# rl-augmented-mpc/Biped-PyMPC

Measured on AMD Instinct MI355X. Metric: batched SRBD QP solves/sec (N=10, 10 PDIPM iters), higher is better.
Workload: dtype f64; 1 GPU; SRBD MPC QP step: qp_former + 10-iteration sparse PDIPM, batch 4096/GPU, horizon N=10, standing gait; batch_per_gpu=4096, global_batch=4096, horizon=10, pdipm_iters=10, refinement=adaptive, parallelism=dp1

## Files before the change

### biped_pympc_amd/_native.py

```python
from __future__ import annotations

import ctypes
import os

from biped_pympc_amd.build import LIB_DIR

_LIB_NAME = "libsrbd_mpc.so"
_lib = None

_c_dp = ctypes.c_void_p


class NativeLibraryMissing(RuntimeError):
    pass


def lib_path() -> str:
    return os.environ.get("SRBD_LIB") or os.path.join(LIB_DIR, _LIB_NAME)


def lib() -> ctypes.CDLL:
    global _lib
    if _lib is not None:
        return _lib
# ... 44 lines not shown
    L.srbd_scratch_pool_slots.restype = ctypes.c_int
    L.srbd_scratch_pool_slots.argtypes = []
    L.srbd_scratch_slot_bytes.restype = ctypes.c_size_t
    L.srbd_scratch_slot_bytes.argtypes = []
    L.srbd_evaluate_qp_former.restype = ctypes.c_float
    L.srbd_evaluate_qp_former.argtypes = [ctypes.c_int, ctypes.c_void_p, ctypes.c_void_p,
                                          ctypes.c_void_p, ctypes.c_int]
    L.srbd_evaluate_pdipm.restype = ctypes.c_float
    L.srbd_evaluate_pdipm.argtypes = [ctypes.c_int, ctypes.c_int, ctypes.c_void_p, ctypes.c_void_p,
                                      ctypes.c_void_p, ctypes.c_int]
    L.srbd_set_solver_path.restype = ctypes.c_int
    L.srbd_set_solver_path.argtypes = [ctypes.c_int]
    L.srbd_get_solver_path.restype = ctypes.c_int
    L.srbd_get_solver_path.argtypes = []
    L.srbd_set_refinement.restype = ctypes.c_int
    L.srbd_set_refinement.argtypes = [ctypes.c_int]
    L.srbd_get_refinement.restype = ctypes.c_int
    L.srbd_get_refinement.argtypes = []
    L.srbd_set_refinement_policy.restype = ctypes.c_int
    L.srbd_set_refinement_policy.argtypes = [ctypes.c_int, ctypes.c_double]
    L.srbd_pattern_ccs.restype = ctypes.c_int
    L.srbd_pattern_ccs.argtypes = [ctypes.c_int, ctypes.c_int, ctypes.POINTER(ctypes.c_int),
                                   ctypes.POINTER(ctypes.c_int)]
    L.srbd_prepare_inputs.restype = ctypes.c_int
    L.srbd_prepare_inputs.argtypes = [ctypes.c_int, ctypes.c_int, ctypes.POINTER(MPCPrep), P, ctypes.c_void_p]
    L.srbd_mpc_step.restype = ctypes.c_int
    L.srbd_mpc_step.argtypes = [ctypes.c_int, ctypes.c_int, ctypes.c_int, ctypes.c_double, ctypes.POINTER(MPCPrep),
                                P, P, _c_dp, ctypes.c_int, _c_dp, _c_dp, _c_dp, ctypes.c_void_p]
    L.srbd_mpc_step_ex.restype = ctypes.c_int
    L.srbd_mpc_step_ex.argtypes = L.srbd_mpc_step.argtypes[:-1] + [_c_dp, ctypes.c_void_p]
    L.srbd_u0_wrench.restype = ctypes.c_int
    L.srbd_u0_wrench.argtypes = [ctypes.c_int, ctypes.c_int, _c_dp, _c_dp, _c_dp, ctypes.c_void_p]
    L.srbd_u0_wrench_torque.restype = ctypes.c_int
    L.srbd_u0_wrench_torque.argtypes = [ctypes.c_int, ctypes.c_int, _c_dp, _c_dp, _c_dp, ctypes.c_int, _c_dp,
                                        _c_dp, _c_dp, ctypes.c_void_p]
    L.srbd_dense_scatter.restype = ctypes.c_int
    L.srbd_dense_scatter.argtypes = [ctypes.c_int, ctypes.c_int, ctypes.c_int, _c_dp, _c_dp, _c_dp,
                                     ctypes.c_void_p]
    _lib = L
    return L


class _Tolerant:

    class _Missing:
        def __init__(self, name):
# ... 153 lines not shown
```

### biped_pympc_amd/csrc/pdipm_srbd_reg.hpp

```cpp
#pragma once
#include "pdipm_srbd.hpp"
#include "qp_former.hpp"
#include "mpc_io.hpp"

#ifndef SRBD_PROGRESS_PRIO
#define SRBD_PROGRESS_PRIO 1
#endif
#ifndef SRBD_PHASE_ATTR
#define SRBD_PHASE_ATTR
#endif
#ifndef SRBD_REFINE_COMBINED
#define SRBD_REFINE_COMBINED 0
#endif
#ifndef SRBD_SWP_INV
#define SRBD_SWP_INV 0
#endif

namespace srbd {

__host__ __device__ constexpr int reg_tpb(int N) { return N <= 10 ? 64 : (N <= 21 ? 128 : (N <= 24 ? 192 : 256)); }
__host__ __device__ constexpr bool reg_horizon(int N) { return N >= 2 && N <= 32; }

template <int TPB>
__device__ __forceinline__ void qp_sync() {
// ... 214 lines not shown
}
template <bool kForce = true>
__device__ __forceinline__ double ncol(const double* nd, int col, const double* v, int p) {
  double a0 = nd[nd_idx(0, col)] * v[0] + nd[nd_idx(1, col)] * v[1];
  double a1 = nd[nd_idx(2, col)] * v[2] + nd[nd_idx(6, col)] * v[6];
  double a2 = nd[nd_idx(7, col)] * v[7] + nd[nd_idx(8, col)] * v[8];
  if (kForce) {
    a0 += nd[nd_idx(3 + p, col)] * v[3 + p];
    a1 += nd[nd_idx(9 + p, col)] * v[9 + p];
  }
  return (a0 + a1) + a2;
}

__host__ __device__ constexpr int g_other(int k) { return k < 2 ? 0 : (k < 4 ? 1 : (k < 6 ? 3 : 0)); }

__host__ __device__ constexpr int g_row(int k) { return 4 * k + kGfPad * (k >> 3); }

__device__ __forceinline__ double grow4(const double* gf, int k, const double* xu) {
  const int f = k >> 3, o = g_other(k & 7);
  const double* g = gf + g_row(k);
  return g[o] * xu[foot_colj(f, o)] + g[2] * xu[foot_colj(f, 2)];
}

template <int N, bool kFReg = true>
struct RegCtx {
  static constexpr int TPB = reg_tpb(N);
  using Lo = RegLayout<N>;
  static constexpr int nz = Lo::nz, m = Lo::m, p = Lo::p, nx = Lo::nx;
  static constexpr int SI = Lo::SI, SE = Lo::SE, SX = Lo::SX;
  static_assert(6 * N <= TPB && 2 * N <= TPB, "equality-row slots");
  struct ERow {
    int e, i, r;
    bool valid;
  };
  __device__ static ERow erow(int l, int t) {
    ERow q;
    if (t == 2) {
      q.valid = l < 2 * N;
      q.e = nx + l;
      q.i = l >> 1;
      q.r = l & 1;
      return q;
    }
    q.valid = l < 6 * N;
    q.i = div6(l);
    const int k = l - m24(q.i, 6);
// ... 66 lines not shown
  }
  __device__ bool block_any_or_all(bool p, bool q) {
    if constexpr (TPB == 64) return __any(p) || !__any(!q);
    else return block_reduce<true>(p ? -1.0 : (q ? 1.0 : 0.0)) != 0.0;
  }
  __device__ double block_min(double v) { return block_reduce<true>(v); }
  __device__ int fresh_lane() const {
    int l = lane;
    asm volatile("" : "+v"(l));
    __builtin_assume(l < TPB);
    return l;
  }
  __device__ static constexpr bool full_slot(int t, int n) { return TPB * (t + 1) <= n; }

  template <int t>
  __device__ double arow(const double* V, const double* Mc, const double* Pd, const double* Nd, const ERow& q) const {
    const double mv = mrow_slot<t>(Mc, q.r, V + 12 * (q.i >= 1 ? q.i - 1 : 0));
    double v = (q.i >= 1 ? 1.0 : 0.0) * mv;
    v += Pd[q.r] * V[12 * q.i + q.r];
    v += nrow<t>(Nd, q.r, V + nx + 12 * q.i);
    return v;
  }
  __device__ static int sink(bool valid, int e, int base) { return valid ? e : Lo::DMY - base; }
  template <int t>
  __device__ void re_slot(const double* X, const double* Mc, const double* Pd, const double* Nd,
                          const double (&bv)[SE]) {
    const ERow q = erow(fresh_lane(), t);
    re[t] = arow<t>(X, Mc, Pd, Nd, q) - bv[t];
  }
  template <int t>
  __device__ void g_slot(const double* TV, const double* Mc, const double* Pd, const double* Nd, double* QV) {
    const ERow q = erow(fresh_lane(), t);
    QV[sink(q.valid, q.e, Lo::QV)] = arow<t>(TV, Mc, Pd, Nd, q) + re[t];
  }
  SRBD_PHASE_ATTR __device__ double residuals(bool want_mu) {
    const int lane = fresh_lane();
    const double *X = at(Lo::X), *Y = at(Lo::Y), *Z = at(Lo::Z), *Mc = at(Lo::Mc), *Nd = at(Lo::Nd),
                 *Gf = at(Lo::Gf), *Pd = at(Lo::Pd), *Hu = at(Lo::Hu), *SG = at(Lo::SG);
    double *RXu = at(Lo::RXu), *REm = at(Lo::REm);
    const double(&fx)[SX] = fxr, (&fu)[SX] = fur, (&bv)[SE] = bvr, (&hv)[SI] = hvr;
#pragma unroll
    for (int t = 0; t < SX; ++t) {
      const int c = lane + TPB * t;
      if (full_slot(t, nx) || c < nx) {
        const int k = div12(c) + 1, j = c - m24(k - 1, 12);
        const double v = Hu[12 + j] * X[c] + ((kFReg || t == 0) ? fx[t] : fg()[c]);
        double ay = Pd[j] * Y[12 * (k - 1) + j];
        const double my = mcol(Mc, j, Y + 12 * (k < N ? k : N - 1));
        ay = fma(k < N ? 1.0 : 0.0, my, ay);
        rxx[t] = v + ay;
      }
    }
#pragma unroll
    for (int t = 0; t < SX; ++t) {
      const int c = lane + TPB * t;
      if (full_slot(t, nx) || c < nx) {
        const int i = div12(c), j = c - m24(i, 12);
        const double v = Hu[j] * X[nx + c] + ((kFReg || t == 0) ? fu[t] : fg()[nx + c]);
        const int fj = foot_of(j), f = fj >= 0 ? fj : 0;
        const double* zf = Z + 16 * i + 8 * f;
        const double* g = Gf + g_row(8 * f) + foot_pos(j);
        double g0 = 0.0, g1 = 0.0;
#pragma unroll
        for (int k = 0; k < 4; ++k) {
          g0 += g[4 * k] * zf[k];
          g1 += g[4 * (k + 4)] * zf[k + 4];
        }
        const double gz = (fj >= 0 ? 1.0 : 0.0) * (g0 + g1);
        double ay = ncol(Nd, j, Y + 12 * i, j % 3);
        const bool e9 = j == 9;
        const double se = (j == 6 || e9) ? 1.0 : 0.0;
        ay = fma(se * (e9 ? SG[7] : SG[6]), Y[nx + 2 * i + (e9 ? 1 : 0)], ay);
        RXu[c] = (v + gz) + ay;
      }
    }
    re_slot<0>(X, Mc, Pd, Nd, bv);
    re_slot<1>(X, Mc, Pd, Nd, bv);
    {
      const ERow q = erow(lane, 2);
      if (q.valid) {
        const int w = q.r;
        re[2] = SG[6 + w] * X[nx + 12 * q.i + (w ? 9 : 6)] - (kFReg ? bv[2] : bg()[q.e]);
        REm[q.e - nx] = re[2];
      }
    }
    double sz = 0.0;
#pragma unroll
    for (int t = 0; t < SI; ++t) {
      const int q = lane + TPB * t;
      if (RegCtx<N>::full_slot(t, m) || q < m) {
        const int i = q >> 4, k = q & 15;
        const double v = grow4(Gf, k, X + nx + m24(i, 12));
        rs[t] = (v + s[t]) - ((kFReg || t < SI - 1) ? hv[t] : hg()[q]);
        sz += s[t] * z[t];
      }
    }
    qp_sync<TPB>();
    return want_mu ? block_sum(sz) / m : 0.0;
  }

  __device__ static double fwd_rhs(bool act, bool prev, bool mstep, int g, int r, const CoupleRow& Cr, double w,
                                   const double* qv) {
    double q = 0.0;
    if (act && !(mstep && g == 1)) q = *qv;
    if (act && prev) q = couple_cw_sub(Cr, w, q);
    if (mstep && nb >= 1) q += __shfl(q, 16 + perm12(r), 64);
    return q;
  }

  __device__ void factor() {
    factor_build();
    factor_chain<false>();
  }

  __device__ void foot_inverse(int fl, double* dst) {
// ... 195 lines not shown
        }
        if constexpr (kFwd) {
          const double q = fwd_rhs(act, prev, mstep, g, r, Cr, wf, QV + 12 * i + pr);
          if (act && !(mstep && g == 1)) {
            wf = dot_bc12(Dr, q);
            QV[12 * i + pr] = wf;
          }
        }
      }
    }
    qp_sync<TPB>();
    PROF_ADD(2);
  }

  template <int kMode>
  __device__ void solve(double smu, bool rx = false, bool step0 = true) {
    solve_rhs<kMode>(smu, rx);
    solve_chain<false>();
    solve_finish<false, false, true>(step0);
  }

  template <int t, bool kPark>
  __device__ void rho_slot(const double* TV, const double* Mc, const double* Pd, const double* Nd, double* QV,
                           double* DYs) {
    const ERow q = erow(fresh_lane(), t);
    const double v = arow<t>(TV, Mc, Pd, Nd, q);
    const int e = sink(q.valid, q.e, Lo::QV);
    const double dy = QV[e];
    if (kPark) DYs[sink(q.valid, q.e, Lo::RXu)] = dy;
    QV[e] = (v + re[t]) - kDelta * dy;
  }
  template <bool kAff = false>
  SRBD_PHASE_ATTR __device__ void refine_rhs(bool row1 = true) {
    const int lane = fresh_lane();
    const double *Mc = at(Lo::Mc), *Nd = at(Lo::Nd), *Pd = at(Lo::Pd), *Gf = at(Lo::Gf), *Hu = at(Lo::Hu);
    double *TV = at(Lo::TV), *QV = at(Lo::QV), *DYs = at(Lo::RXu), *Zd = at(Lo::Z);
    if constexpr (kAff) {
      double *VV = at(Lo::VV);
#pragma unroll
      for (int t = 0; t < SI; ++t) {
        const int q = lane + TPB * t;
        e3r[t] = 0.0;
        if (RegCtx<N>::full_slot(t, m) || q < m) {
          const int i = q >> 4, k = q & 15;
          const double gd = grow4(Gf, k, TV + nx + m24(i, 12));
          const double e3 = -rs[t] - ((gd + ds[t]) - kDelta * dz[t]);
          const double e2 = Zd[q] - (wd[t] * ds[t] + dz[t]);
          const double qc = di[t] * (e2 - wd[t] * e3);
          VV[q] = VV[q] + qc;
          e3r[t] = e3;
          Zd[q] = dz[t] + qc;
        }
      }
    }
    qp_sync<TPB>();
    const int fl = lane;
    if (row1 && (unsigned)fl < 2u * N) {
      const int i = fl >> 1, f = fl & 1, b = 12 * i;
      const double* zf = Zd + 16 * i + 8 * f;
      const double* RXu = DYs;
      const double* g = Gf + g_row(8 * f);
      double gt[4];
      {
        double zk[8];
#pragma unroll
        for (int k = 0; k < 8; ++k) zk[k] = zf[k];
        gt[0] = g[0] * zk[0] + g[4] * zk[1];
        gt[1] = g[9] * zk[2] + g[13] * zk[3];
// ... 3 lines not shown
        for (int k = 0; k < 4; ++k) {
          gz0 += g[4 * k + 2] * zk[k];
          gz1 += g[4 * (k + 4) + 2] * zk[k + 4];
        }
        gt[2] = gz0 + gz1;
      }
      double e1[4], c[4];
#pragma unroll
      for (int a = 0; a < 4; ++a) {
        const int j = foot_colj(f, a);
        const double ay = a < 3 ? ncol(Nd, j, QV + b, a) : ncol<false>(Nd, j, QV + b, 0);
        e1[a] = ((-RXu[b + j] - (Hu[j] + kBeta) * TV[nx + b + j]) - gt[a]) - ay;
      }
      phi_solve(fl, e1, c);
#pragma unroll
      for (int a = 0; a < 4; ++a) TV[nx + b + foot_colj(f, a)] += c[a];
    }
    qp_sync<TPB>();
    if (kAff) {
#pragma unroll
      for (int t = 0; t < SI; ++t)
        if (full_slot(t, m) || lane + TPB * t < m) Zd[lane + TPB * t] = e3r[t];
    }
    rho_slot<0, !kAff>(TV, Mc, Pd, Nd, QV, DYs);
    rho_slot<1, !kAff>(TV, Mc, Pd, Nd, QV, DYs);
    qp_sync<TPB>();
    PROF_ADD(6);
  }

  template <int kMode>
  SRBD_PHASE_ATTR __device__ void solve_rhs(double smu, bool rx = false) {
    const int lane = fresh_lane();
    double *VV = at(Lo::VV), *TV = at(Lo::TV), *QV = at(Lo::QV), *Zr2 = at(Lo::Z);
    const double *RXu = at(Lo::RXu), *REm = at(Lo::REm), *IX = at(Lo::IX), *Gf = at(Lo::Gf),
                 *SG = at(Lo::SG), *Mc = at(Lo::Mc), *Nd = at(Lo::Nd), *Pd = at(Lo::Pd);
#pragma unroll
    for (int t = 0; t < SI; ++t) {
      const int q = lane + TPB * t;
      if (RegCtx<N>::full_slot(t, m) || q < m) {
        const double si = rcp3(s[t]);
        double r2 = -(si * (s[t] * z[t]));
        if (kMode == 1) r2 = r2 + -(si * (s[t] * z[t] + ds[t] * dz[t] - smu));
        Zr2[q] = r2;
        VV[q] = di[t] * (r2 + wd[t] * rs[t]);
      }
    }
#pragma unroll
    for (int t = 0; t < SX; ++t) {
      const int c = lane + TPB * t;
      if ((kMode == 0 || rx) && (full_slot(t, nx) || c < nx)) TV[c] = -rxx[t] * IX[c - m24(div12(c), 12)];
    }
    qp_sync<TPB>();
    rhs_tasks<kMode>(lane, rx);
    qp_sync<TPB>();
    g_slot<0>(TV, Mc, Pd, Nd, QV);
    g_slot<1>(TV, Mc, Pd, Nd, QV);
    qp_sync<TPB>();
    PROF_ADD(3);
  }

  template <int kMode>
  __device__ void rhs_tasks(int fl, bool rx) {
    double* TV = at(Lo::TV);
    const double *VV = at(Lo::VV), *RXu = at(Lo::RXu), *REm = at(Lo::REm), *Gf = at(Lo::Gf), *SG = at(Lo::SG);
    if ((unsigned)fl < (unsigned)(((kMode == 0 || rx) ? 3 : 2) * N)) {
      if (fl < 2 * N) {
        const int i = fl >> 1, f = fl & 1, b = 12 * i;
        double rv[4], tv[4];
        {
          const double* vv = VV + 16 * i + 8 * f;
          const double* g = Gf + g_row(8 * f);
          double vk[8];
#pragma unroll
          for (int k = 0; k < 8; ++k) vk[k] = vv[k];
          const double gfx = g[0] * vk[0] + g[4] * vk[1];
          const double gfy = g[9] * vk[2] + g[13] * vk[3];
          const double gmy = g[19] * vk[4] + g[23] * vk[5];
          double gz0 = 0.0, gz1 = 0.0;
#pragma unroll
// ... 85 lines not shown
      }
#pragma unroll
      for (int te = T - 1; te >= 0; --te) {
        if (te < cnt) {
          const int i = g ? N - 1 - te : te;
          double Dr[12];
#pragma unroll
          for (int k = 0; k < 12; ++k) Dr[k] = dv_at(DV, offs[k], 2 * kDvBytes * te);
          y = dot_bc12_sub(Dr, couple_cty2(Ct, y), wv[te]);
          if (own) QV[12 * i + pr] = y;
        }
      }
    }
    qp_sync<TPB>();
    PROF_ADD(4);
  }

  template <bool kRefine = false, bool kAffine = false, bool kStep0 = false>
  SRBD_PHASE_ATTR __device__ void solve_finish(bool step0 = true) {
    const int lane = fresh_lane();
    double *VV = at(Lo::VV), *TV = at(Lo::TV), *QV = at(Lo::QV), *DYm = at(Lo::DYm);
    const double *RXu = at(Lo::RXu), *REm = at(Lo::REm), *IX = at(Lo::IX), *Gf = at(Lo::Gf),
                 *SG = at(Lo::SG), *Mc = at(Lo::Mc), *Nd = at(Lo::Nd), *Pd = at(Lo::Pd);
#pragma unroll
    for (int t = 0; t < SX; ++t) {
      const int c = lane + TPB * t;
      if (!kAffine && (full_slot(t, nx) || c < nx)) {
        const int k = div12(c) + 1, j = c - m24(k - 1, 12);
        double aty = Pd[j] * QV[12 * (k - 1) + j];
        const double mq = mcol(Mc, j, QV + 12 * (k < N ? k : N - 1));
        aty = fma(k < N ? 1.0 : 0.0, mq, aty);
        TV[c] = TV[c] - aty * IX[j];
      }
    }
    const int fl = lane;
    if ((unsigned)fl < (unsigned)((kAffine ? 2 : 3) * N)) {
      const bool foot = kAffine || fl < 2 * N;
      const int i = foot ? (fl >> 1) : fl - 2 * N;
      const int b = nx + 12 * i;
      const double* yi = QV + 12 * i;
      if (foot) {
        const int f = fl & 1;
        double av[4], tv[4];
#pragma unroll
        for (int a = 0; a < 3; ++a) av[a] = ncol(Nd, foot_colj(f, a), yi, a);
        av[3] = ncol<false>(Nd, foot_colj(f, 3), yi, 0);
        phi_solve(fl, av, tv);
#pragma unroll
        for (int a = 0; a < 4; ++a) {
          const int o = b + foot_colj(f, a);
          TV[o] = TV[o] - tv[a];
        }
      } else {
        const double r4a = kRefine ? 0.0 : -REm[2 * i], r4b = kRefine ? 0.0 : -REm[2 * i + 1];
        const double a6 = ncol<false>(Nd, 6, yi, 0), a9 = ncol<false>(Nd, 9, yi, 0);
        const double a8 = ncol<false>(Nd, 8, yi, 0), a11 = ncol<false>(Nd, 11, yi, 0);
        TV[b + 6] -= SG[0] * a6;
        TV[b + 9] -= SG[2] * a9;
        TV[b + 8] -= SG[1] * a8;
        TV[b + 11] -= SG[3] * a11;
        if constexpr (kRefine) {
          DYm[2 * i] -= (SG[6] * a6) * SG[8];
          DYm[2 * i + 1] -= (SG[7] * a9) * SG[9];
        } else {
          const double rho6 = -RXu[12 * i + 6] - a6, rho9 = -RXu[12 * i + 9] - a9;
          DYm[2 * i] = (SG[6] * rho6 - SG[4] * r4a) * SG[8];
          DYm[2 * i + 1] = (SG[7] * rho9 - SG[5] * r4b) * SG[9];
        }
      }
    }
    qp_sync<TPB>();
#pragma unroll
    for (int t = 0; t < SI; ++t) {
      const int q = lane + TPB * t;
      if (RegCtx<N>::full_slot(t, m) || q < m) {
        const int i = q >> 4, k = q & 15;
        const double gd = grow4(Gf, k, TV + nx + m24(i, 12));
        const double vq = VV[q];
        dz[t] = vq + di[t] * wd[t] * gd;
        const double r3 = (kRefine && kAffine) ? at(Lo::Z)[q] - rs[t] : -rs[t];
        ds[t] = r3 - gd + kDelta * dz[t];
        if (kStep0 && step0) {
          double* Zd = at(Lo::Z);
          const double e3 = -rs[t] - ((gd + ds[t]) - kDelta * dz[t]);
          const double e2 = Zd[q] - (wd[t] * ds[t] + dz[t]);
          const double qc = di[t] * (e2 - wd[t] * e3);
          VV[q] = vq + qc;
          rs[t] = rs[t] - e3;
          Zd[q] = dz[t] + qc;
        }
      }
    }
    PROF_ADD(3);
  }

  __device__ double step_length(const double (&v)[SI], const double (&dv)[SI]) {
    const int lane = fresh_lane();
    double mn = INFINITY;
#pragma unroll
    for (int t = 0; t < SI; ++t) {
// ... 526 lines not shown
```

### biped_pympc_amd/csrc/srbd_mpc.hip

```cpp
#include <hip/hip_runtime.h>

#include <algorithm>
#include <cstdio>
#include <cstdlib>
#include <cstring>
#include <mutex>
#include <shared_mutex>
#include <string>
#include <vector>

#include "../../include/srbd_mpc.h"
#include "pdipm.hpp"
#include "pdipm_srbd.hpp"
#include "pdipm_srbd_reg.hpp"
#include "mpc_step_lds.hpp"
#include "qp_former.hpp"
#include "mpc_io.hpp"
#include "reg20.hpp"
#include "regN.hpp"
#include "device_state.hpp"

#ifndef SRBD_BUILD_ID
#define SRBD_BUILD_ID "0000000000000000"
#endif
// ... 226 lines not shown
  Events* ev = events.at(current_device());
  if (!ev) {
    set_error((int)hipErrorInvalidDevice, "no current HIP device (or index >= 64)");
    return -1.0f;
  }
  if (!ev->ev[0]) {
    if (hipEventCreate(&ev->ev[0]) != hipSuccess || hipEventCreate(&ev->ev[1]) != hipSuccess) {
      set_error((int)hipErrorInitializationError, "hipEventCreate");
      return -1.0f;
    }
  }
  (void)hipEventRecord(ev->ev[0], 0);
  if (launch() != 0) return -1.0f;
  (void)hipEventRecord(ev->ev[1], 0);
  hipError_t e = hipEventSynchronize(ev->ev[1]);
  if (e == hipSuccess) e = hipDeviceSynchronize();
  if (e != hipSuccess) {
    set_error((int)e, "kernel execution");
    return -1.0f;
  }
  float ms = 0.0f;
  (void)hipEventElapsedTime(&ms, ev->ev[0], ev->ev[1]);
  return ms / 1000.0f;
}

}

extern "C" {

int srbd_abi_version(void) { return SRBD_ABI_VERSION; }

const char* srbd_build_id(void) { return kBuildIdTag + sizeof("srbd-build-id:") - 1; }

const char* srbd_last_error(void) { return g_last_error.c_str(); }

size_t srbd_solver_lds_bytes(int horizon) { return horizon_ok(horizon) ? solver_lds_bytes(horizon) : 0; }

int srbd_set_solver_path(int path) {
  if (path < 0 || path > 2)
    return set_error(kErrInvalid, "srbd_set_solver_path: 0 (auto), 1 (general) or 2 (LDS-resident fast)");
  int* p = g_solver_path.at(current_device());
  if (!p) return set_error((int)hipErrorInvalidDevice, "srbd_set_solver_path: no current HIP device");
  *p = path;
  return 0;
}

// ... 311 lines not shown
      a.prep.out[i] = former_inputs[i];
    }
  a.ctrl = 1;
  if (outputs)
    for (int i = 0; i < 6; ++i) a.out[i] = outputs[i];
  a.wrench = foot_wrench;
  a.tau = tau;
  a.jac = contact_jacobian;
  a.contact = contact_bool;
  a.ndof = tau ? ndof : 0;
  a.N = horizon;
  a.n_iter = n_iter;
  a.batch = batch;
  a.y0 = y0;
  a.status = status;
  return launch_step(a, (hipStream_t)stream);
}

int srbd_mpc_step(int horizon, int n_iter, int batch, double y0, const srbd_mpc_prep* prep,
                  double* const* former_inputs, double* const* outputs, float* foot_wrench, int ndof,
                  const float* contact_jacobian, const float* contact_bool, float* tau, void* stream) {
  return srbd_mpc_step_ex(horizon, n_iter, batch, y0, prep, former_inputs, outputs, foot_wrench, ndof,
                          contact_jacobian, contact_bool, tau, nullptr, stream);
}

int srbd_pattern_ccs(int horizon, int which, int* colptr, int* rowind) {
  if (!horizon_ok(horizon) || !colptr || !rowind) return -1;
  constexpr srbd::Tables T = srbd::make_tables();
  const int N = horizon, nz = 24 * N;
  int nnz = 0;
  std::vector<int> row, col;
  auto put = [&](int off, int r, int c) {
    if (off < 0 || off >= nnz) return false;
    if (row[off] != -1) return false;
    row[off] = r;
    col[off] = c;
    return true;
  };
  if (which == 0) {
    nnz = nz;
    row.assign(nnz, -1);
    col.assign(nnz, -1);
    for (int c = 0; c < nz; ++c)
      if (!put(c, c, c)) return -2;
  } else if (which == 1) {
    nnz = srbd::nnz_A(N);
// ... 89 lines not shown
```

### include/srbd_mpc.h

```cpp
#ifndef SRBD_MPC_H_
#define SRBD_MPC_H_

#include <stddef.h>

#ifdef __cplusplus
extern "C" {
#endif

#define SRBD_ABI_VERSION 1
#define SRBD_MAX_HORIZON 32

float evaluate(const double* inputs[], double* work, double* outputs[], const int batch_size);

int srbd_abi_version(void);
const char* srbd_last_error(void);
const char* srbd_build_id(void);

float srbd_evaluate_qp_former(int horizon, const double* inputs[], double* work, double* outputs[],
                              int batch);
float srbd_evaluate_pdipm(int horizon, int n_iter, const double* inputs[], double* work,
                          double* outputs[], int batch);

int srbd_qp_former(int horizon, int batch, const double* const* inputs, double* const* outputs,
                   void* stream);
// ... 29 lines not shown
int srbd_get_solver_path(void);

int srbd_set_refinement(int mode);
int srbd_get_refinement(void);

#define SRBD_REFINE_AFFINE_ALL 1
#define SRBD_REFINE_AFFINE_AT_INIT 2
#define SRBD_REFINE_AFFINE_FIRST(k) (((k) & 255) << 8)
#define SRBD_REFINE_AFFINE_LAST(k) (((k) & 255) << 16)
int srbd_set_refinement_policy(int flags, double w);

int srbd_prepare_device(void);

int srbd_release_device(void);

int srbd_set_scratch_slots(int slots);

size_t srbd_scratch_pool_bytes(void);
int srbd_scratch_pool_slots(void);
size_t srbd_scratch_slot_bytes(void);

int srbd_pattern_ccs(int horizon, int which, int* colptr, int* rowind);


typedef struct srbd_mpc_prep {
  const float* root_euler;
  const float* root_position;
  const float* root_angular_velocity_w;
  const float* root_velocity_w;
  const float* rotation_body;
  const float* foot_position;
  const float* desired_velocity_b;
  const float* desired_angular_velocity_b;
  const float* desired_height;
  float* world_position_desired;
  float* yaw_desired;
  unsigned char* first_run;
  const float* gait_phase;
  const int* ssp_durations;
  const int* dsp_durations;
  const float* contact_table;
  const float* dt_mpc;
  const float* residual_lin_accel;
  const float* residual_ang_accel;
  float I_body[9];
  double mass, mu;
// ... 34 lines not shown
```

Before: 6.747 million solves/s.

## Replace per-lane index arithmetic with constant-memory byte-offset lane tables

```diff
diff --git a/biped_pympc_amd/_native.py b/biped_pympc_amd/_native.py
--- a/biped_pympc_amd/_native.py
+++ b/biped_pympc_amd/_native.py
@@ -90,6 +90,8 @@
     L.srbd_pattern_ccs.restype = ctypes.c_int
     L.srbd_pattern_ccs.argtypes = [ctypes.c_int, ctypes.c_int, ctypes.POINTER(ctypes.c_int),
                                    ctypes.POINTER(ctypes.c_int)]
+    L.srbd_lane_table.restype = ctypes.c_int
+    L.srbd_lane_table.argtypes = [ctypes.c_int, ctypes.c_int, ctypes.POINTER(ctypes.c_uint), ctypes.c_int]
     L.srbd_prepare_inputs.restype = ctypes.c_int
     L.srbd_prepare_inputs.argtypes = [ctypes.c_int, ctypes.c_int, ctypes.POINTER(MPCPrep), P, ctypes.c_void_p]
     L.srbd_mpc_step.restype = ctypes.c_int
diff --git a/biped_pympc_amd/csrc/pdipm_srbd_reg.hpp b/biped_pympc_amd/csrc/pdipm_srbd_reg.hpp
--- a/biped_pympc_amd/csrc/pdipm_srbd_reg.hpp
+++ b/biped_pympc_amd/csrc/pdipm_srbd_reg.hpp
@@ -260,6 +260,267 @@
   return g[o] * xu[foot_colj(f, o)] + g[2] * xu[foot_colj(f, 2)];
 }
 
+#ifndef SRBD_LANE_TABLES
+#define SRBD_LANE_TABLES 1
+#endif
+
+__device__ __forceinline__ double lds_off(const double* base, uint32_t off) {
+  return *reinterpret_cast<const double*>(reinterpret_cast<const char*>(base) + off);
+}
+__device__ __forceinline__ double& lds_off(double* base, uint32_t off) {
+  return *reinterpret_cast<double*>(reinterpret_cast<char*>(base) + off);
+}
+
+constexpr int kGRowTabRows = 16 * 32;
+struct GRowTab {
+  alignas(16) uint32_t o[kGRowTabRows][4];
+};
+__host__ __device__ constexpr uint32_t grow_ref(int q, int w) {
+  const int i = q >> 4, k = q & 15, f = k >> 3, o = g_other(k & 7);
+  return (uint32_t)(8 * (w == 0 ? g_row(k) + o : (w == 1 ? g_row(k) + 2 : 12 * i + foot_colj(f, w == 2 ? o : 2))));
+}
+constexpr GRowTab make_grow_tab() {
+  GRowTab t{};
+  int q = 0;
+  for (int i = 0; i < 32; ++i)
+    for (int f = 0; f < 2; ++f)
+      for (int k = 0; k < 8; ++k, ++q) {
+        const int row = 4 * (8 * f + k) + kGfPad * f;
+        const int oth = k < 2 ? 0 : (k < 4 ? 1 : (k < 6 ? 3 : 0));
+        const int co = oth < 3 ? oth + 3 * f : 7 + 3 * f, cz = 2 + 3 * f;
+        t.o[q][0] = (uint32_t)(8 * (row + oth));
+        t.o[q][1] = (uint32_t)(8 * (row + 2));
+        t.o[q][2] = (uint32_t)(8 * (12 * i + co));
+        t.o[q][3] = (uint32_t)(8 * (12 * i + cz));
+      }
+  return t;
+}
+constexpr bool grow_tab_ok() {
+  const GRowTab t = make_grow_tab();
+  for (int q = 0; q < kGRowTabRows; ++q)
+    for (int w = 0; w < 4; ++w)
+      if (t.o[q][w] != grow_ref(q, w)) return false;
+  return true;
+}
+static_assert(grow_tab_ok(), "c_growtab differs from grow4's index arithmetic");
+static __constant__ GRowTab c_growtab = make_grow_tab();
+
+template <class T>
+__device__ __forceinline__ T ctab_load(const void* base, uint32_t off) {
+  return *reinterpret_cast<const T*>(reinterpret_cast<const char*>(base) + off);
+}
+__device__ __forceinline__ double grow4_tab(const double* gf, const uint4& o, const double* u) {
+  return lds_off(gf, o.x) * lds_off(u, o.z) + lds_off(gf, o.y) * lds_off(u, o.w);
+}
+
+constexpr uint32_t kOneHi = 0x3FF0u;
+
+constexpr int kUColTabRows = 12 * 32 + 128;
+struct UColTab {
+  alignas(16) uint32_t a[kUColTabRows][4];
+  alignas(16) uint32_t b[kUColTabRows][4];
+  alignas(16) uint32_t c[kUColTabRows][4];
+};
+__host__ __device__ constexpr uint32_t ucol_ref(int c, int w) {
+  const int i = c / 12, j = c % 12;
+  const int fj = (j < 3 || j == 7) ? 0 : ((j < 6 || j == 10) ? 1 : -1), f = fj >= 0 ? fj : 0;
+  const int pos = j < 6 ? j % 3 : 3, p = j % 3, e9 = j == 9 ? 1 : 0;
+  switch (w) {
+    case 0: return (uint32_t)(8 * j);
+    case 1: return (uint32_t)(8 * 12 * i);
+    case 2: return (uint32_t)(8 * (16 * i + 8 * f));
+    case 3: return (uint32_t)(8 * (g_row(8 * f) + pos));
+    case 4: return (uint32_t)(8 * nd_idx(3 + p, j));
+    case 5: return (uint32_t)(8 * (12 * i + 3 + p));
+    case 6: return ((fj >= 0 ? kOneHi : 0u) << 16) | ((j == 6 || j == 9) ? kOneHi : 0u);
+    case 7: return 0u;
+    case 8: return (uint32_t)(8 * (6 + e9));
+    default: return (uint32_t)(8 * (2 * i + e9));
+  }
+}
+constexpr UColTab make_ucol_tab() {
+  UColTab tb{};
+  constexpr int foot[12] = {0, 0, 0, 1, 1, 1, -1, 0, -1, -1, 1, -1}, posn[12] = {0, 1, 2, 0, 1, 2, 3, 3, 3, 3, 3, 3},
+                m3[12] = {0, 1, 2, 0, 1, 2, 0, 1, 2, 0, 1, 2};
+  int i = 0, j = 0;
+  for (int c = 0; c < kUColTabRows; ++c) {
+    const int f = foot[j] > 0 ? 1 : 0;
+    tb.a[c][0] = (uint32_t)(8 * j);
+    tb.a[c][1] = (uint32_t)(96 * i);
+    tb.a[c][2] = (uint32_t)(128 * i + 64 * f);
+    tb.a[c][3] = (uint32_t)(8 * ((32 + kGfPad) * f + posn[j]));
+    tb.b[c][0] = (uint32_t)(8 * (kNdS * (3 + m3[j]) + j));
+    tb.b[c][1] = (uint32_t)(96 * i + 24 + 8 * m3[j]);
+    tb.b[c][2] = (foot[j] >= 0 ? kOneHi << 16 : 0u) | ((j == 6 || j == 9) ? kOneHi : 0u);
+    tb.b[c][3] = 0u;
+    tb.c[c][0] = (uint32_t)(j == 9 ? 56 : 48);
+    tb.c[c][1] = (uint32_t)(16 * i + (j == 9 ? 8 : 0));
+    if (++j == 12) {
+      j = 0;
+      ++i;
+    }
+  }
+  return tb;
+}
+constexpr bool ucol_tab_ok() {
+  const UColTab tb = make_ucol_tab();
+  for (int c = 0; c < kUColTabRows; ++c)
+    for (int w = 0; w < 10; ++w)
+      if ((w < 4 ? tb.a[c][w] : (w < 8 ? tb.b[c][w - 4] : tb.c[c][w - 8])) != ucol_ref(c, w)) return false;
+  return true;
+}
+static_assert(ucol_tab_ok(), "c_ucoltab differs from the u-column pass's index arithmetic");
+static __constant__ UColTab c_ucoltab = make_ucol_tab();
+struct UColOffs {
+  uint4 a, b;
+  uint2 c;
+};
+
+template <int N>
+struct ERowTab {
+  static constexpr int TPB = reg_tpb(N);
+  alignas(16) uint32_t a[2][TPB][4];
+  alignas(16) uint32_t b[2][TPB][4];
+  alignas(16) uint32_t c[2][TPB][4];
+};
+template <int N>
+__host__ __device__ constexpr uint32_t erow_ref(int l, int t, int w) {
+  using Lo = RegLayout<N>;
+  const int i = l / 6, k = l % 6, ip = i >= 1 ? i - 1 : 0;
+  const int r = t == 0 ? (k < 3 ? k : k + 3) : (k < 3 ? k + 3 : k + 6);
+  const int rr = t == 0 ? (r < 3 ? r : 0) : (r < 6 ? r : 3);
+  const bool valid = l < 6 * N, ws = t == 0 ? r < 3 : r < 6;
+  const int e = 12 * i + r;
+  switch (w) {
+    case 0: return (uint32_t)(8 * e);
+    case 1: return (uint32_t)(8 * (12 * ip + r));
+    case 2: return (uint32_t)(8 * (12 * ip + (t == 0 ? 0 : rr + 6)));
+    case 3: return (uint32_t)(8 * (12 * i + (t == 0 ? 0 : r % 3)));
+    case 4: return (uint32_t)(8 * r);
+    case 5: return (uint32_t)(8 * (t == 0 ? 12 + 3 * rr : 21 + rr - 3));
+    case 6: return (uint32_t)(8 * nd_idx(r, t == 0 ? 0 : r % 3));
+    case 7: return ((i >= 1 ? kOneHi : 0u) << 16) | (ws ? kOneHi : 0u);
+    case 8: return (uint32_t)(8 * (valid ? e : Lo::DMY - Lo::QV));
+    default: return (uint32_t)(8 * (valid ? e : Lo::DMY - Lo::RXu));
+  }
+}
+template <int N>
+constexpr ERowTab<N> make_erow_tab() {
+  using Lo = RegLayout<N>;
+  ERowTab<N> tb{};
+  for (int t = 0; t < 2; ++t) {
+    int i = 0, k = 0;
+    for (int l = 0; l < ERowTab<N>::TPB; ++l) {
+      const int r = (k < 3 ? k : k + 3) + 3 * t;
+      const int p3 = k < 3 ? k : k - 3;
+      const bool ws = k < 3;
+      const int rr = ws ? r : 3 * t;
+      const int vi = 96 * i, vp = i >= 1 ? vi - 96 : 0;
+      tb.a[t][l][0] = (uint32_t)(vi + 8 * r);
+      tb.a[t][l][1] = (uint32_t)(vp + 8 * r);
+      tb.a[t][l][2] = (uint32_t)(vp + (t == 0 ? 0 : 8 * (rr + 6)));
+      tb.a[t][l][3] = (uint32_t)(vi + (t == 0 ? 0 : 8 * p3));
+      tb.b[t][l][0] = (uint32_t)(8 * r);
+      tb.b[t][l][1] = (uint32_t)(t == 0 ? 96 + 24 * rr : 8 * (18 + rr));
+      tb.b[t][l][2] = (uint32_t)(8 * kNdS * r + (t == 0 ? 0 : 8 * p3));
+      tb.b[t][l][3] = ((i >= 1 ? kOneHi : 0u) << 16) | (ws ? kOneHi : 0u);
+      const bool valid = i < N;
+      tb.c[t][l][0] = valid ? tb.a[t][l][0] : (uint32_t)(8 * (Lo::DMY - Lo::QV));
+      tb.c[t][l][1] = valid ? tb.a[t][l][0] : (uint32_t)(8 * (Lo::DMY - Lo::RXu));
+      if (++k == 6) {
+        k = 0;
+        ++i;
+      }
+    }
+  }
+  return tb;
+}
+template <int N>
+constexpr bool erow_tab_ok() {
+  const ERowTab<N> tb = make_erow_tab<N>();
+  for (int t = 0; t < 2; ++t)
+    for (int l = 0; l < ERowTab<N>::TPB; ++l)
+      for (int w = 0; w < 10; ++w) {
+        const uint32_t v = w < 4 ? tb.a[t][l][w] : (w < 8 ? tb.b[t][l][w - 4] : tb.c[t][l][w - 8]);
+        if (v != erow_ref<N>(l, t, w)) return false;
+      }
+  return true;
+}
+template <int N>
+struct ERowTabHolder {
+  static_assert(erow_tab_ok<N>(), "c_erowtab differs from erow / arow / sink's index arithmetic");
+  static constexpr ERowTab<N> value = make_erow_tab<N>();
+};
+template <int N>
+static __constant__ ERowTab<N> c_erowtab = ERowTabHolder<N>::value;
+
+struct ERowOffs {
+  uint4 a, b;
+  uint2 c;
+};
+
+template <int N>
+struct XColTab {
+  static constexpr int TPB = reg_tpb(N), rows = TPB * RegLayout<N>::SX;
+  alignas(16) uint32_t a[rows][4];
+  alignas(16) uint32_t b[rows][4];
+};
+template <int N>
+__host__ __device__ constexpr uint32_t xcol_ref(int c, int w) {
+  const int k = c / 12 + 1, j = c - 12 * (k - 1), kc = k < N ? k : N - 1;
+  const bool b6 = j >= 6 && j < 9, b9 = j >= 9;
+  const int j6 = b6 ? j - 6 : 0, j9 = b9 ? j - 9 : 0;
+  switch (w) {
+    case 0: return (uint32_t)(8 * j);
+    case 1: return (uint32_t)(8 * (12 * kc + j));
+    case 2: return (uint32_t)(8 * 12 * kc);
+    case 3: return (uint32_t)(8 * (12 * kc + j9 + 3));
+    case 4: return (uint32_t)(8 * j6);
+    case 5: return (uint32_t)(8 * j9);
+    case 6: return ((b6 ? kOneHi : 0u) << 16) | (b9 ? kOneHi : 0u);
+    default: return (k < N ? kOneHi : 0u) << 16;
+  }
+}
+template <int N>
+constexpr XColTab<N> make_xcol_tab() {
+  XColTab<N> tb{};
+  int s = 0, j = 0;
+  for (int c = 0; c < XColTab<N>::rows; ++c) {
+    const int vk = 96 * (s + 1 < N ? s + 1 : N - 1);
+    tb.a[c][0] = (uint32_t)(8 * j);
+    tb.a[c][1] = (uint32_t)(vk + 8 * j);
+    tb.a[c][2] = (uint32_t)vk;
+    tb.a[c][3] = (uint32_t)(vk + (j >= 9 ? 8 * (j - 6) : 24));
+    tb.b[c][0] = (uint32_t)(j >= 6 && j < 9 ? 8 * (j - 6) : 0);
+    tb.b[c][1] = (uint32_t)(j >= 9 ? 8 * (j - 9) : 0);
+    tb.b[c][2] = j >= 9 ? kOneHi : (j >= 6 ? kOneHi << 16 : 0u);
+    tb.b[c][3] = s + 1 < N ? kOneHi << 16 : 0u;
+    if (++j == 12) {
+      j = 0;
+      ++s;
+    }
+  }
+  return tb;
+}
+template <int N>
+constexpr bool xcol_tab_ok() {
+  const XColTab<N> tb = make_xcol_tab<N>();
+  for (int c = 0; c < XColTab<N>::rows; ++c)
+    for (int w = 0; w < 8; ++w)
+      if ((w < 4 ? tb.a[c][w] : tb.b[c][w - 4]) != xcol_ref<N>(c, w)) return false;
+  return true;
+}
+template <int N>
+struct XColTabHolder {
+  static_assert(xcol_tab_ok<N>(), "c_xcoltab differs from the x-column passes' index arithmetic");
+  static constexpr XColTab<N> value = make_xcol_tab<N>();
+};
+template <int N>
+static __constant__ XColTab<N> c_xcoltab = XColTabHolder<N>::value;
+struct XColOffs {
+  uint4 a, b;
+};
+
 template <int N, bool kFReg = true>
 struct RegCtx {
   static constexpr int TPB = reg_tpb(N);
@@ -372,16 +633,90 @@
     return v;
   }
   __device__ static int sink(bool valid, int e, int base) { return valid ? e : Lo::DMY - base; }
+  static constexpr bool kTab = SRBD_LANE_TABLES != 0 && TPB == 64;
+  template <bool kSink>
+  __device__ static ERowOffs load_erow(int l, int t) {
+    const uint32_t off = (uint32_t)l * 16u;
+    ERowOffs o;
+    o.a = ctab_load<uint4>(c_erowtab<N>.a[t], off);
+    o.b = ctab_load<uint4>(c_erowtab<N>.b[t], off);
+    if constexpr (kSink) o.c = ctab_load<uint2>(c_erowtab<N>.c[t], off);
+    else o.c = make_uint2(0u, 0u);
+    return o;
+  }
+  __device__ static uint4 load_grow(int l, int t) {
+    static_assert(TPB * SI <= kGRowTabRows, "c_growtab covers every slot of every lane");
+    return ctab_load<uint4>(c_growtab.o[TPB * t], (uint32_t)l * 16u);
+  }
+  __device__ static XColOffs load_xcol(int l, int t) {
+    const uint32_t off = (uint32_t)l * 16u;
+    return {ctab_load<uint4>(c_xcoltab<N>.a[TPB * t], off), ctab_load<uint4>(c_xcoltab<N>.b[TPB * t], off)};
+  }
+  __device__ static UColOffs load_ucol(int l, int t) {
+    static_assert(TPB * SX <= kUColTabRows, "c_ucoltab covers every slot of every lane");
+    const uint32_t off = (uint32_t)l * 16u;
+    return {ctab_load<uint4>(c_ucoltab.a[TPB * t], off), ctab_load<uint4>(c_ucoltab.b[TPB * t], off),
+            ctab_load<uint2>(c_ucoltab.c[TPB * t], off)};
+  }
+  template <bool kHi>
+  __device__ static double tab_weight(uint32_t w) {
+    return __hiloint2double((int)(kHi ? w & 0xFFFF0000u : w << 16), 0);
+  }
+  __device__ static double mcol_tab(const double* Mc, const double* V, const XColOffs& o) {
+    const double a = lds_off(Mc, o.a.x) * lds_off(V, o.a.y);
+    const double x6 = (lds_off(Mc + 12, o.b.x) * lds_off(V, o.a.z) + lds_off(Mc + 15, o.b.x) * lds_off(V + 1, o.a.z)) +
+                      lds_off(Mc + 18, o.b.x) * lds_off(V + 2, o.a.z);
+    const double x9 = lds_off(Mc + 21, o.b.y) * lds_off(V, o.a.w);
+    return fma(tab_weight<false>(o.b.z), x9, fma(tab_weight<true>(o.b.z), x6, a));
+  }
+  template <int t>
+  __device__ static double arow_tab(const double* V, const double* Mc, const double* Pd, const double* Nd,
+                                    const ERowOffs& o) {
+    const double wi = tab_weight<true>(o.b.w), ws = tab_weight<false>(o.b.w);
+    const double a = lds_off(Mc, o.b.x) * lds_off(V, o.a.y);
+    double x;
+    if constexpr (t == 0)
+      x = (lds_off(Mc, o.b.y) * lds_off(V + 6, o.a.z) + lds_off(Mc + 1, o.b.y) * lds_off(V + 7, o.a.z)) +
+          lds_off(Mc + 2, o.b.y) * lds_off(V + 8, o.a.z);
+    else
+      x = lds_off(Mc, o.b.y) * lds_off(V, o.a.z);
+    const double mv = fma(ws, x, a);
+    double v = wi * mv;
+    v += lds_off(Pd, o.b.x) * lds_off(V, o.a.x);
+    const double* U = V + nx;
+    if constexpr (t == 0) {
+      double a0 = 0.0, a1 = 0.0, a2 = 0.0;
+#pragma unroll
+      for (int j = 0; j < 4; ++j) {
+        a0 += lds_off(Nd + j, o.b.z) * lds_off(U + j, o.a.w);
+        a1 += lds_off(Nd + j + 4, o.b.z) * lds_off(U + j + 4, o.a.w);
+        a2 += lds_off(Nd + j + 8, o.b.z) * lds_off(U + j + 8, o.a.w);
+      }
+      v += (a0 + a1) + a2;
+    } else {
+      v += lds_off(Nd, o.b.z) * lds_off(U, o.a.w) + lds_off(Nd + 3, o.b.z) * lds_off(U + 3, o.a.w);
+    }
+    return v;
+  }
   template <int t>
   __device__ void re_slot(const double* X, const double* Mc, const double* Pd, const double* Nd,
-                          const double (&bv)[SE]) {
-    const ERow q = erow(fresh_lane(), t);
-    re[t] = arow<t>(X, Mc, Pd, Nd, q) - bv[t];
+                          const double (&bv)[SE], const ERowOffs& o) {
+    if constexpr (kTab) {
+      re[t] = arow_tab<t>(X, Mc, Pd, Nd, o) - bv[t];
+    } else {
+      const ERow q = erow(fresh_lane(), t);
+      re[t] = arow<t>(X, Mc, Pd, Nd, q) - bv[t];
+    }
   }
   template <int t>
-  __device__ void g_slot(const double* TV, const double* Mc, const double* Pd, const double* Nd, double* QV) {
-    const ERow q = erow(fresh_lane(), t);
-    QV[sink(q.valid, q.e, Lo::QV)] = arow<t>(TV, Mc, Pd, Nd, q) + re[t];
+  __device__ void g_slot(const double* TV, const double* Mc, const double* Pd, const double* Nd, double* QV,
+                         const ERowOffs& o) {
+    if constexpr (kTab) {
+      lds_off(QV, o.c.x) = arow_tab<t>(TV, Mc, Pd, Nd, o) + re[t];
+    } else {
+      const ERow q = erow(fresh_lane(), t);
+      QV[sink(q.valid, q.e, Lo::QV)] = arow<t>(TV, Mc, Pd, Nd, q) + re[t];
+    }
   }
   SRBD_PHASE_ATTR __device__ double residuals(bool want_mu) {
     const int lane = fresh_lane();
@@ -389,22 +724,67 @@
                  *Gf = at(Lo::Gf), *Pd = at(Lo::Pd), *Hu = at(Lo::Hu), *SG = at(Lo::SG);
     double *RXu = at(Lo::RXu), *REm = at(Lo::REm);
     const double(&fx)[SX] = fxr, (&fu)[SX] = fur, (&bv)[SE] = bvr, (&hv)[SI] = hvr;
+    XColOffs xo[SX];
+    UColOffs uo[SX];
+    ERowOffs eo[2];
+    uint4 go[SI];
+    if constexpr (kTab) {
+#pragma unroll
+      for (int t = 0; t < SX; ++t) xo[t] = load_xcol(lane, t);
+#pragma unroll
+      for (int t = 0; t < SX; ++t) uo[t] = load_ucol(lane, t);
+#pragma unroll
+      for (int t = 0; t < 2; ++t) eo[t] = load_erow<false>(lane, t);
+#pragma unroll
+      for (int t = 0; t < SI; ++t) go[t] = load_grow(lane, t);
+    }
 #pragma unroll
     for (int t = 0; t < SX; ++t) {
       const int c = lane + TPB * t;
       if (full_slot(t, nx) || c < nx) {
-        const int k = div12(c) + 1, j = c - m24(k - 1, 12);
-        const double v = Hu[12 + j] * X[c] + ((kFReg || t == 0) ? fx[t] : fg()[c]);
-        double ay = Pd[j] * Y[12 * (k - 1) + j];
-        const double my = mcol(Mc, j, Y + 12 * (k < N ? k : N - 1));
-        ay = fma(k < N ? 1.0 : 0.0, my, ay);
-        rxx[t] = v + ay;
+        if constexpr (kTab) {
+          const double v = lds_off(Hu + 12, xo[t].a.x) * X[c] + ((kFReg || t == 0) ? fx[t] : fg()[c]);
+          double ay = lds_off(Pd, xo[t].a.x) * Y[c];
+          const double my = mcol_tab(Mc, Y, xo[t]);
+          ay = fma(tab_weight<true>(xo[t].b.w), my, ay);
+          rxx[t] = v + ay;
+        } else {
+          const int k = div12(c) + 1, j = c - m24(k - 1, 12);
+          const double v = Hu[12 + j] * X[c] + ((kFReg || t == 0) ? fx[t] : fg()[c]);
+          double ay = Pd[j] * Y[12 * (k - 1) + j];
+          const double my = mcol(Mc, j, Y + 12 * (k < N ? k : N - 1));
+          ay = fma(k < N ? 1.0 : 0.0, my, ay);
+          rxx[t] = v + ay;
+        }
       }
     }
 #pragma unroll
     for (int t = 0; t < SX; ++t) {
       const int c = lane + TPB * t;
-      if (full_slot(t, nx) || c < nx) {
+      if constexpr (kTab) {
+        if (full_slot(t, nx) || c < nx) {
+          const UColOffs& o = uo[t];
+          const double v = lds_off(Hu, o.a.x) * X[nx + c] + ((kFReg || t == 0) ? fu[t] : fg()[nx + c]);
+          double g0 = 0.0, g1 = 0.0;
+#pragma unroll
+          for (int k = 0; k < 4; ++k) {
+            g0 += lds_off(Gf + 4 * k, o.a.w) * lds_off(Z + k, o.a.z);
+            g1 += lds_off(Gf + 4 * (k + 4), o.a.w) * lds_off(Z + k + 4, o.a.z);
+          }
+          const double gz = tab_weight<true>(o.b.z) * (g0 + g1);
+          double a0 = lds_off(Nd + nd_idx(0, 0), o.a.x) * lds_off(Y, o.a.y) +
+                      lds_off(Nd + nd_idx(1, 0), o.a.x) * lds_off(Y + 1, o.a.y);
+          double a1 = lds_off(Nd + nd_idx(2, 0), o.a.x) * lds_off(Y + 2, o.a.y) +
+                      lds_off(Nd + nd_idx(6, 0), o.a.x) * lds_off(Y + 6, o.a.y);
+          const double a2 = lds_off(Nd + nd_idx(7, 0), o.a.x) * lds_off(Y + 7, o.a.y) +
+                            lds_off(Nd + nd_idx(8, 0), o.a.x) * lds_off(Y + 8, o.a.y);
+          a0 += lds_off(Nd, o.b.x) * lds_off(Y, o.b.y);
+          a1 += lds_off(Nd + nd_idx(6, 0), o.b.x) * lds_off(Y + 6, o.b.y);
+          double ay = (a0 + a1) + a2;
+          ay = fma(tab_weight<false>(o.b.z) * lds_off(SG, o.c.x), lds_off(Y + nx, o.c.y), ay);
+          RXu[c] = (v + gz) + ay;
+        }
+      } else if (full_slot(t, nx) || c < nx) {
         const int i = div12(c), j = c - m24(i, 12);
         const double v = Hu[j] * X[nx + c] + ((kFReg || t == 0) ? fu[t] : fg()[nx + c]);
         const int fj = foot_of(j), f = fj >= 0 ? fj : 0;
@@ -424,8 +804,8 @@
         RXu[c] = (v + gz) + ay;
       }
     }
-    re_slot<0>(X, Mc, Pd, Nd, bv);
-    re_slot<1>(X, Mc, Pd, Nd, bv);
+    re_slot<0>(X, Mc, Pd, Nd, bv, eo[0]);
+    re_slot<1>(X, Mc, Pd, Nd, bv, eo[1]);
     {
       const ERow q = erow(lane, 2);
       if (q.valid) {
@@ -439,8 +819,13 @@
     for (int t = 0; t < SI; ++t) {
       const int q = lane + TPB * t;
       if (RegCtx<N>::full_slot(t, m) || q < m) {
-        const int i = q >> 4, k = q & 15;
-        const double v = grow4(Gf, k, X + nx + m24(i, 12));
+        double v;
+        if constexpr (kTab) {
+          v = grow4_tab(Gf, go[t], X + nx);
+        } else {
+          const int i = q >> 4, k = q & 15;
+          v = grow4(Gf, k, X + nx + m24(i, 12));
+        }
         rs[t] = (v + s[t]) - ((kFReg || t < SI - 1) ? hv[t] : hg()[q]);
         sz += s[t] * z[t];
       }
@@ -682,19 +1067,31 @@
 
   template <int t, bool kPark>
   __device__ void rho_slot(const double* TV, const double* Mc, const double* Pd, const double* Nd, double* QV,
-                           double* DYs) {
-    const ERow q = erow(fresh_lane(), t);
-    const double v = arow<t>(TV, Mc, Pd, Nd, q);
-    const int e = sink(q.valid, q.e, Lo::QV);
-    const double dy = QV[e];
-    if (kPark) DYs[sink(q.valid, q.e, Lo::RXu)] = dy;
-    QV[e] = (v + re[t]) - kDelta * dy;
+                           double* DYs, const ERowOffs& o) {
+    if constexpr (kTab) {
+      const double v = arow_tab<t>(TV, Mc, Pd, Nd, o);
+      const double dy = lds_off(QV, o.c.x);
+      if (kPark) lds_off(DYs, o.c.y) = dy;
+      lds_off(QV, o.c.x) = (v + re[t]) - kDelta * dy;
+    } else {
+      const ERow q = erow(fresh_lane(), t);
+      const double v = arow<t>(TV, Mc, Pd, Nd, q);
+      const int e = sink(q.valid, q.e, Lo::QV);
+      const double dy = QV[e];
+      if (kPark) DYs[sink(q.valid, q.e, Lo::RXu)] = dy;
+      QV[e] = (v + re[t]) - kDelta * dy;
+    }
   }
   template <bool kAff = false>
   SRBD_PHASE_ATTR __device__ void refine_rhs(bool row1 = true) {
     const int lane = fresh_lane();
     const double *Mc = at(Lo::Mc), *Nd = at(Lo::Nd), *Pd = at(Lo::Pd), *Gf = at(Lo::Gf), *Hu = at(Lo::Hu);
     double *TV = at(Lo::TV), *QV = at(Lo::QV), *DYs = at(Lo::RXu), *Zd = at(Lo::Z);
+    ERowOffs eo[2];
+    if constexpr (kTab) {
+#pragma unroll
+      for (int t = 0; t < 2; ++t) eo[t] = load_erow<true>(lane, t);
+    }
     if constexpr (kAff) {
       double *VV = at(Lo::VV);
 #pragma unroll
@@ -702,8 +1099,13 @@
         const int q = lane + TPB * t;
         e3r[t] = 0.0;
         if (RegCtx<N>::full_slot(t, m) || q < m) {
-          const int i = q >> 4, k = q & 15;
-          const double gd = grow4(Gf, k, TV + nx + m24(i, 12));
+          double gd;
+          if constexpr (kTab) {
+            gd = grow4_tab(Gf, load_grow(lane, t), TV + nx);
+          } else {
+            const int i = q >> 4, k = q & 15;
+            gd = grow4(Gf, k, TV + nx + m24(i, 12));
+          }
           const double e3 = -rs[t] - ((gd + ds[t]) - kDelta * dz[t]);
           const double e2 = Zd[q] - (wd[t] * ds[t] + dz[t]);
           const double qc = di[t] * (e2 - wd[t] * e3);
@@ -753,8 +1155,8 @@
       for (int t = 0; t < SI; ++t)
         if (full_slot(t, m) || lane + TPB * t < m) Zd[lane + TPB * t] = e3r[t];
     }
-    rho_slot<0, !kAff>(TV, Mc, Pd, Nd, QV, DYs);
-    rho_slot<1, !kAff>(TV, Mc, Pd, Nd, QV, DYs);
+    rho_slot<0, !kAff>(TV, Mc, Pd, Nd, QV, DYs, eo[0]);
+    rho_slot<1, !kAff>(TV, Mc, Pd, Nd, QV, DYs, eo[1]);
     qp_sync<TPB>();
     PROF_ADD(6);
   }
@@ -765,6 +1167,15 @@
     double *VV = at(Lo::VV), *TV = at(Lo::TV), *QV = at(Lo::QV), *Zr2 = at(Lo::Z);
     const double *RXu = at(Lo::RXu), *REm = at(Lo::REm), *IX = at(Lo::IX), *Gf = at(Lo::Gf),
                  *SG = at(Lo::SG), *Mc = at(Lo::Mc), *Nd = at(Lo::Nd), *Pd = at(Lo::Pd);
+    ERowOffs eo[2];
+    uint32_t xj[SX];
+    if constexpr (kTab) {
+#pragma unroll
+      for (int t = 0; t < SX; ++t)
+        if (kMode == 0 || rx) xj[t] = ctab_load<uint32_t>(c_xcoltab<N>.a[TPB * t], (uint32_t)lane * 16u);
+#pragma unroll
+      for (int t = 0; t < 2; ++t) eo[t] = load_erow<true>(lane, t);
+    }
 #pragma unroll
     for (int t = 0; t < SI; ++t) {
       const int q = lane + TPB * t;
@@ -779,13 +1190,14 @@
 #pragma unroll
     for (int t = 0; t < SX; ++t) {
       const int c = lane + TPB * t;
-      if ((kMode == 0 || rx) && (full_slot(t, nx) || c < nx)) TV[c] = -rxx[t] * IX[c - m24(div12(c), 12)];
+      if ((kMode == 0 || rx) && (full_slot(t, nx) || c < nx))
+        TV[c] = -rxx[t] * (kTab ? lds_off(IX, xj[t]) : IX[c - m24(div12(c), 12)]);
     }
     qp_sync<TPB>();
     rhs_tasks<kMode>(lane, rx);
     qp_sync<TPB>();
-    g_slot<0>(TV, Mc, Pd, Nd, QV);
-    g_slot<1>(TV, Mc, Pd, Nd, QV);
+    g_slot<0>(TV, Mc, Pd, Nd, QV, eo[0]);
+    g_slot<1>(TV, Mc, Pd, Nd, QV, eo[1]);
     qp_sync<TPB>();
     PROF_ADD(3);
   }
@@ -917,15 +1329,31 @@
     double *VV = at(Lo::VV), *TV = at(Lo::TV), *QV = at(Lo::QV), *DYm = at(Lo::DYm);
     const double *RXu = at(Lo::RXu), *REm = at(Lo::REm), *IX = at(Lo::IX), *Gf = at(Lo::Gf),
                  *SG = at(Lo::SG), *Mc = at(Lo::Mc), *Nd = at(Lo::Nd), *Pd = at(Lo::Pd);
+    XColOffs xo[SX];
+    uint4 go[SI];
+    if constexpr (kTab) {
+#pragma unroll
+      for (int t = 0; t < SX; ++t)
+        if (!kAffine) xo[t] = load_xcol(lane, t);
+#pragma unroll
+      for (int t = 0; t < SI; ++t) go[t] = load_grow(lane, t);
+    }
 #pragma unroll
     for (int t = 0; t < SX; ++t) {
       const int c = lane + TPB * t;
       if (!kAffine && (full_slot(t, nx) || c < nx)) {
-        const int k = div12(c) + 1, j = c - m24(k - 1, 12);
-        double aty = Pd[j] * QV[12 * (k - 1) + j];
-        const double mq = mcol(Mc, j, QV + 12 * (k < N ? k : N - 1));
-        aty = fma(k < N ? 1.0 : 0.0, mq, aty);
-        TV[c] = TV[c] - aty * IX[j];
+        if constexpr (kTab) {
+          double aty = lds_off(Pd, xo[t].a.x) * QV[c];
+          const double mq = mcol_tab(Mc, QV, xo[t]);
+          aty = fma(tab_weight<true>(xo[t].b.w), mq, aty);
+          TV[c] = TV[c] - aty * lds_off(IX, xo[t].a.x);
+        } else {
+          const int k = div12(c) + 1, j = c - m24(k - 1, 12);
+          double aty = Pd[j] * QV[12 * (k - 1) + j];
+          const double mq = mcol(Mc, j, QV + 12 * (k < N ? k : N - 1));
+          aty = fma(k < N ? 1.0 : 0.0, mq, aty);
+          TV[c] = TV[c] - aty * IX[j];
+        }
       }
     }
     const int fl = lane;
@@ -969,8 +1397,13 @@
     for (int t = 0; t < SI; ++t) {
       const int q = lane + TPB * t;
       if (RegCtx<N>::full_slot(t, m) || q < m) {
-        const int i = q >> 4, k = q & 15;
-        const double gd = grow4(Gf, k, TV + nx + m24(i, 12));
+        double gd;
+        if constexpr (kTab) {
+          gd = grow4_tab(Gf, go[t], TV + nx);
+        } else {
+          const int i = q >> 4, k = q & 15;
+          gd = grow4(Gf, k, TV + nx + m24(i, 12));
+        }
         const double vq = VV[q];
         dz[t] = vq + di[t] * wd[t] * gd;
         const double r3 = (kRefine && kAffine) ? at(Lo::Z)[q] - rs[t] : -rs[t];
diff --git a/biped_pympc_amd/csrc/srbd_mpc.hip b/biped_pympc_amd/csrc/srbd_mpc.hip
--- a/biped_pympc_amd/csrc/srbd_mpc.hip
+++ b/biped_pympc_amd/csrc/srbd_mpc.hip
@@ -272,6 +272,23 @@
   float ms = 0.0f;
   (void)hipEventElapsedTime(&ms, ev->ev[0], ev->ev[1]);
   return ms / 1000.0f;
+}
+
+template <int kN>
+void lane_table_words(int N, int which, std::vector<unsigned>& w) {
+  if constexpr (kN <= 32) {
+    if (N != kN) return lane_table_words<kN + 1>(N, which, w);
+    if (which == 1) {
+      static constexpr srbd::ERowTab<kN> T = srbd::make_erow_tab<kN>();
+      for (int t = 0; t < 2; ++t)
+        for (int l = 0; l < srbd::ERowTab<kN>::TPB; ++l)
+          for (int k = 0; k < 10; ++k) w.push_back(k < 4 ? T.a[t][l][k] : (k < 8 ? T.b[t][l][k - 4] : T.c[t][l][k - 8]));
+    } else {
+      static constexpr srbd::XColTab<kN> T = srbd::make_xcol_tab<kN>();
+      for (int c = 0; c < srbd::XColTab<kN>::rows; ++c)
+        for (int k = 0; k < 8; ++k) w.push_back(k < 4 ? T.a[c][k] : T.b[c][k - 4]);
+    }
+  }
 }
 
 }
@@ -629,6 +646,25 @@
                   const float* contact_jacobian, const float* contact_bool, float* tau, void* stream) {
   return srbd_mpc_step_ex(horizon, n_iter, batch, y0, prep, former_inputs, outputs, foot_wrench, ndof,
                           contact_jacobian, contact_bool, tau, nullptr, stream);
+}
+
+int srbd_lane_table(int horizon, int which, unsigned* out, int cap) {
+  std::vector<unsigned> w;
+  if (which == 0) {
+    static constexpr srbd::GRowTab T = srbd::make_grow_tab();
+    for (int q = 0; q < srbd::kGRowTabRows; ++q)
+      for (int k = 0; k < 4; ++k) w.push_back(T.o[q][k]);
+  } else if (which == 3) {
+    static constexpr srbd::UColTab T = srbd::make_ucol_tab();
+    for (int c = 0; c < srbd::kUColTabRows; ++c)
+      for (int k = 0; k < 10; ++k) w.push_back(k < 4 ? T.a[c][k] : (k < 8 ? T.b[c][k - 4] : T.c[c][k - 8]));
+  } else if ((which == 1 || which == 2) && srbd::reg_horizon(horizon)) {
+    lane_table_words<2>(horizon, which, w);
+  } else {
+    return -1;
+  }
+  for (int k = 0; k < (int)w.size() && k < cap && out; ++k) out[k] = w[k];
+  return (int)w.size();
 }
 
 int srbd_pattern_ccs(int horizon, int which, int* colptr, int* rowind) {
diff --git a/include/srbd_mpc.h b/include/srbd_mpc.h
--- a/include/srbd_mpc.h
+++ b/include/srbd_mpc.h
@@ -75,6 +75,8 @@
 
 int srbd_pattern_ccs(int horizon, int which, int* colptr, int* rowind);
 
+int srbd_lane_table(int horizon, int which, unsigned* out, int cap);
+
 
 typedef struct srbd_mpc_prep {
   const float* root_euler;
```

Result: no change. 6.791 million solves/s (median of 6 runs) (+0.6%).
